# zzuiekongning/MGDT-YOLO

Measured on AMD Instinct MI355X. Metric: images/sec @640x640 bs=32 per GPU, detection forward + NMS (whole job: 1 GPU(s)), higher is better.
Workload: dtype bf16; 1 GPU; mspa_c2f_gd_yolov8-n (MSPA-C2f + GD neck + Detect, nc=80) 640x640 inference, batch 32/GPU: forward + decode + NMS(conf 0.25, iou 0.7), hipGraph replay, 4 batches in flight (one captured graph per resident batch, replayed round-robin on 4 streams); global_batch=32, parallelism=replicas x1 (batch-sharded, no data-path collective), rccl_ranks=1, input=bfloat16 NCHW images, 8 different batches resident in HBM (600 MiB) cycled, detections_last_step=9600, weights=seeded random init (no checkpoints offline), batches_in_flight=4

## Files before the change

### include/mgdt.h

```cpp
#ifndef MGDT_H
#define MGDT_H
#include <stddef.h>
#include <stdint.h>

#ifdef __cplusplus
extern "C" {
#endif

typedef void* mgdt_stream;

typedef enum { MGDT_OK = 0, MGDT_BAD_SHAPE = -1, MGDT_BAD_DTYPE = -2, MGDT_LAUNCH_FAIL = -3, MGDT_BAD_ARG = -4,
               MGDT_WORKSPACE = -5 } mgdt_status;
typedef enum { MGDT_F32 = 0, MGDT_BF16 = 1, MGDT_U8 = 2  } mgdt_dtype;
typedef enum { MGDT_ACT_NONE = 0, MGDT_ACT_SILU = 1, MGDT_ACT_RELU = 2, MGDT_ACT_GELU = 3 } mgdt_act;

typedef struct {
  void* p;
  int32_t n, h, w, c;
  int64_t sn, sh, sw, sc;
} mgdt_view;

const char* mgdt_last_error(void);
const char* mgdt_version(void);

// ... 4 lines not shown
int mgdt_conv_pack_dgrad(const float* w_oihw, int cin, int cout, int k, int phase, int dtype, void* packed_out, float* bias_out, mgdt_stream s);
typedef struct mgdt_pack_desc {
  const float* w; const float* conv_bias; const float* bn_gamma; const float* bn_beta; const float* bn_mean; const float* bn_var;
  float bn_eps; int32_t cin, cout, k, dtype, mode;
  void* packed; float* bias_out;
} mgdt_pack_desc;
int mgdt_conv_pack_batch(const mgdt_pack_desc* descs, int n, mgdt_stream s);

int mgdt_conv2d_fwd(const mgdt_view* x, const mgdt_view* x2, const float* in_scale, const float* in_shift,
                    const void* packed_w, const float* bias, int k, int stride, int act, const mgdt_view* r1,
                    const mgdt_view* r2, const mgdt_view* y, int dtype, mgdt_stream s);
size_t mgdt_conv_packed_bytes_fp8(int cin, int cout, int k);
int mgdt_conv_pack_fp8(const float* w_oihw, const float* conv_bias, const float* bn_gamma, const float* bn_beta, const float* bn_mean,
                       const float* bn_var, float bn_eps, int cin, int cout, int k, float x_qscale, void* packed_out, float* bias_out,
                       float* oscale_out, mgdt_stream s);
int mgdt_conv2d_fp8_fwd(const mgdt_view* x, const mgdt_view* x2, const float* in_scale, const float* in_shift, const void* packed_w,
                        const float* bias, const float* oscale, float x_qscale, int k, int stride, int act, const mgdt_view* r1,
                        const mgdt_view* r2, const mgdt_view* y, mgdt_stream s);
enum { MGDT_ROUTE_X2 = 1, MGDT_ROUTE_IN_SCALE = 2, MGDT_ROUTE_IN_SHIFT = 4, MGDT_ROUTE_R1 = 8, MGDT_ROUTE_R2 = 16, MGDT_ROUTE_FP8 = 32 };
enum { MGDT_ROUTE_IGEMM = 0, MGDT_ROUTE_LDS3X3 = 1 };
typedef struct {
  int32_t family, nchunks, waves, lds_bytes;
  int32_t NT, MT, D, extra, nseg, seg_chunks, gx, gy, numTiles, ragged;
  int32_t NBW, tile_rows, ncg, nwg, ntiles;
} mgdt_conv_route;
int mgdt_conv2d_route(const mgdt_view* x, const mgdt_view* y, int k, int stride, int dtype, int flags, int act, mgdt_conv_route* out);
int mgdt_conv2d_phase_fwd(const mgdt_view* x, const void* packed_w, const float* bias, int phase, const mgdt_view* r1, const mgdt_view* r2,
                          const mgdt_view* y, int dtype, mgdt_stream s);

size_t mgdt_cnx_mlp_packed_bytes(int c, int dtype);
int mgdt_cnx_mlp_pack(const float* w1, const float* b1, const float* w2, const float* b2, int c, void* packed, int dtype, mgdt_stream s);
size_t mgdt_cnx_mlp_workspace_bytes(int n, int h, int w, int c);
int mgdt_cnx_mlp_fwd(const mgdt_view* t, const mgdt_view* res, const void* packed, const float* gamma, const float* beta, void* ws,
                     const mgdt_view* y, int dtype, mgdt_stream s);

int mgdt_cnx_block_supported(int n, int h, int w, int c, int dtype);
size_t mgdt_cnx_block_workspace_bytes(int n, int h, int w, int c);
int mgdt_cnx_block_geometry(int h, int w, int c, int* out);
int mgdt_cnx_block_fwd(const mgdt_view* x, const float* dw_w49c, const float* dw_b, const float* ln_w, const float* ln_b, float eps, const void* packed,
                       const float* gamma, const float* beta, const void* tail_w, const float* tail_b, int tail_act, void* ws, size_t ws_bytes,
                       const mgdt_view* y, int dtype, mgdt_stream s);

size_t mgdt_stem2_packed_bytes(void);
int mgdt_stem2_pack(const float* w_folded, void* packed, mgdt_stream s);
int mgdt_stem2_fwd(const mgdt_view* x, int x_dtype, const void* packed0, const float* bias0, const void* packed1, const float* bias1,
                   const mgdt_view* y, mgdt_stream s);
int mgdt_stem2_geometry(int n, int h, int w, int cu_count, int* out);
int mgdt_stem2_route(const mgdt_view* x, int x_dtype, const mgdt_view* y, int cu_count, int* out);

int mgdt_detect_tail_supported(int c2, int c3, int nc, int reg_max, int dtype);
int mgdt_detect_tail_fwd(const mgdt_view* tb, const mgdt_view* tc, const void* wb, const float* bb, const void* wc, const float* bc, int nc,
                         float stride, int a_off, int a_total, const mgdt_view* feat, float* y, unsigned long long* best_keys,
                         const void* wb3, const float* bb3, mgdt_stream s);
int mgdt_detect_tail_aug_fwd(const mgdt_view* tb, const mgdt_view* tc, const void* wb, const float* bb, const void* wc, const float* bc, int nc,
                             float stride, int a_off, int a_total, const mgdt_view* feat, float* y, unsigned long long* best_keys,
                             const void* wb3, const float* bb3, float aug_scale, int aug_flip, float aug_img_w, mgdt_stream s);

int mgdt_scale_img_fwd(const mgdt_view* x, int x_dtype, int flip, int hs, int ws, float pad, const mgdt_view* y, int y_dtype, mgdt_stream s);

int mgdt_csp_block_supported(int mode, int cin, int cout, int wd, int nbtl, int h, int w, int dtype);
int mgdt_csp_block_tiles(int mode, int n, int cin, int cout, int wd, int nbtl, int h, int w, int* geom8);
int mgdt_csp_block_fwd(int mode, const mgdt_view* x, const void* front, const float* front_bias, const void* const* mid,
                       const float* const* mid_bias, int nbtl, int shortcut, const void* back, const float* back_bias, int wd, int act,
                       const mgdt_view* y, float* pool, int dtype, mgdt_stream s);

size_t mgdt_pw_chain_packed_bytes(int wd, int dtype);
int mgdt_pw_chain_pack(int idx, const float* w_oi, const float* conv_bias, const float* bn_gamma, const float* bn_beta, const float* bn_mean,
                       const float* bn_var, float bn_eps, int wd, int dtype, void* packed, mgdt_stream s);
int mgdt_pw_chain3_fwd(const mgdt_view* x, const void* packed, int wd, int act, const mgdt_view* y, int dtype, mgdt_stream s);

int mgdt_conv1x1_inject_supported(int cin, int cout, int h, int w, int hg, int wg, int dtype);
int mgdt_conv1x1_inject_fwd(const mgdt_view* x, const void* packed_w, const float* bias, const mgdt_view* ga, const mgdt_view* gf,
                            const mgdt_view* y, int dtype, mgdt_stream s);

int mgdt_conv1x1_inject_conv_supported(int cin, int cmid, int cout2, int h, int w, int hg, int wg, int dtype);
int mgdt_conv1x1_inject_conv_fwd(const mgdt_view* x, const void* packed_w, const float* bias, const mgdt_view* ga, const mgdt_view* gf,
                                 const mgdt_view* gsrc, const void* packed_wg, const float* bias_g, int cmid,
                                 const void* packed_w2, const float* bias2, int act2, const mgdt_view* y2, int dtype, mgdt_stream s);

size_t mgdt_groupnorm_workspace_bytes(int n, int c);
int mgdt_groupnorm_fwd(const mgdt_view* x, const float* gamma, const float* beta, int groups, float eps, int act, void* ws, const mgdt_view* y,
                       int dtype, mgdt_stream s);
int mgdt_tood_layer_attn_fwd(const float* sums, int n, int c, int hw, const float* w1, const float* b1, const float* w2, const float* b2, int hid,
                             int stacked, float* scale, mgdt_stream s);
int mgdt_dcnv2_fwd(const mgdt_view* x, const mgdt_view* offset_mask, const float* w_gemm, const float* bias, const mgdt_view* y, int dtype,
                   mgdt_stream s);
int mgdt_dcnv2_mfma_fwd(const mgdt_view* x, const mgdt_view* offset_mask, const void* packed_w, const mgdt_view* y, int dtype, mgdt_stream s);
int mgdt_pixel_gate_fwd(const mgdt_view* x, const mgdt_view* gate, const mgdt_view* y, int dtype, mgdt_stream s);

int mgdt_conv_pack_direct(const float* w_oihw, const float* conv_bias, const float* bn_gamma, const float* bn_beta,
                          const float* bn_mean, const float* bn_var, float bn_eps, int cin_g, int cout, int k,
                          float* w_out, float* bias_out, mgdt_stream s);
int mgdt_conv2d_direct_fwd(const mgdt_view* x, int x_dtype, const float* w_gemm, const float* bias, int k, int stride,
                           int groups, int act, const mgdt_view* y, int dtype, mgdt_stream s);
enum { MGDT_DIRECT_STEM = 0, MGDT_DIRECT_GENERIC = 1, MGDT_DIRECT_REFUSED = 2 };
int mgdt_conv2d_direct_route(const mgdt_view* x, int x_dtype, const mgdt_view* y, int dtype, int k, int stride, int groups, int* out);

#define MGDT_SPR_SPLITS 16
int mgdt_spr_pool_fwd(const mgdt_view* x, float* pooled, int dtype, mgdt_stream s);
int mgdt_spr_attn_fwd(const float* pooled, const float* fc1_w, const float* fc1_b, const float* fc2_w,
                      const float* fc2_b, int n, int c, int groups, int h, int w, int softmax, float* attn, mgdt_stream s);
int mgdt_scale_channels_fwd(const mgdt_view* x, const float* attn, const mgdt_view* y, int dtype, mgdt_stream s);
int mgdt_spr_attn_scale_fwd(const float* pooled, int nsplit, int tiles_x, int tiles_y, const float* fc1_w, const float* fc1_b, const float* fc2_w, const float* fc2_b, int groups,
                            const mgdt_view* x, const mgdt_view* y, const mgdt_view* pool_a, const mgdt_view* pool_b, int dtype, mgdt_stream s);

int mgdt_sppf_pool_fwd(const mgdt_view* x, const mgdt_view* y1, const mgdt_view* y2, const mgdt_view* y3, int dtype,
// ... 234 lines not shown
```

### mgdt_yolo_amd/_lib.py

```python
import ctypes as C
import os

_HERE = os.path.dirname(os.path.abspath(__file__))
LIB_PATH = os.environ.get('MGDT_LIB') or os.path.join(_HERE, 'csrc', 'libmgdt_hip.so')

F32, BF16 = 0, 1
ACT_NONE, ACT_SILU, ACT_RELU, ACT_GELU = 0, 1, 2, 3
SPR_SPLITS = 16
GRN_SPLITS = 8


class View(C.Structure):
    _fields_ = [('p', C.c_void_p), ('n', C.c_int32), ('h', C.c_int32), ('w', C.c_int32), ('c', C.c_int32),
                ('sn', C.c_int64), ('sh', C.c_int64), ('sw', C.c_int64), ('sc', C.c_int64)]


VP = C.POINTER(View)
_vp, _i, _f, _sz, _l = C.c_void_p, C.c_int, C.c_float, C.c_size_t, C.c_long

class PackDesc(C.Structure):
    _fields_ = [('w', C.c_void_p), ('conv_bias', C.c_void_p), ('bn_gamma', C.c_void_p), ('bn_beta', C.c_void_p), ('bn_mean', C.c_void_p), ('bn_var', C.c_void_p),
                ('bn_eps', C.c_float), ('cin', C.c_int32), ('cout', C.c_int32), ('k', C.c_int32), ('dtype', C.c_int32), ('mode', C.c_int32),
                ('packed', C.c_void_p), ('bias_out', C.c_void_p)]


class WgradFinalDesc(C.Structure):
    _fields_ = [('partial', C.c_void_p), ('dw', C.c_void_p), ('n', C.c_long), ('nsplit', C.c_int32), ('accumulate', C.c_int32)]


class ConvRoute(C.Structure):
    _fields_ = [(n, C.c_int32) for n in ('family', 'nchunks', 'waves', 'lds_bytes', 'NT', 'MT', 'D', 'extra', 'nseg', 'seg_chunks', 'gx', 'gy', 'numTiles',
                                         'ragged', 'NBW', 'tile_rows', 'ncg', 'nwg', 'ntiles')]


ROUTE_X2, ROUTE_IN_SCALE, ROUTE_IN_SHIFT, ROUTE_R1, ROUTE_R2, ROUTE_FP8 = 1, 2, 4, 8, 16, 32
ROUTE_IGEMM, ROUTE_LDS3X3 = 0, 1
DIRECT_STEM, DIRECT_GENERIC, DIRECT_REFUSED = 0, 1, 2

PROTOTYPES = {
    'mgdt_last_error': (C.c_char_p, []),
    'mgdt_version': (C.c_char_p, []),
    'mgdt_conv_packed_bytes': (_sz, [_i, _i, _i, _i]),
    'mgdt_conv_pack': (_i, [_vp, _vp, _vp, _vp, _vp, _vp, _f, _i, _i, _i, _i, _vp, _vp, _vp]),
    'mgdt_conv2d_fwd': (_i, [VP, VP, _vp, _vp, _vp, _vp, _i, _i, _i, VP, VP, VP, _i, _vp]),
    'mgdt_conv_packed_bytes_fp8': (_sz, [_i, _i, _i]),
    'mgdt_conv_pack_fp8': (_i, [_vp, _vp, _vp, _vp, _vp, _vp, _f, _i, _i, _i, _f, _vp, _vp, _vp, _vp]),
    'mgdt_conv2d_fp8_fwd': (_i, [VP, VP, _vp, _vp, _vp, _vp, _vp, _f, _i, _i, _i, VP, VP, VP, _vp]),
    'mgdt_conv2d_route': (_i, [VP, VP, _i, _i, _i, _i, _i, C.POINTER(ConvRoute)]),
    'mgdt_conv_pack_batch': (_i, [_vp, _i, _vp]),
    'mgdt_conv2d_phase_fwd': (_i, [VP, _vp, _vp, _i, VP, VP, VP, _i, _vp]),
    'mgdt_conv_wgrad_splits': (_i, [_i, _i, _i]),
    'mgdt_wgrad_final_batch': (_i, [_vp, _i, _vp]),
    'mgdt_conv_pack_dgrad': (_i, [_vp, _i, _i, _i, _i, _i, _vp, _vp, _vp]),
    'mgdt_conv_pack_direct': (_i, [_vp, _vp, _vp, _vp, _vp, _vp, _f, _i, _i, _i, _vp, _vp, _vp]),
    'mgdt_conv2d_direct_fwd': (_i, [VP, _i, _vp, _vp, _i, _i, _i, _i, VP, _i, _vp]),
    'mgdt_conv2d_direct_route': (_i, [VP, _i, VP, _i, _i, _i, _i, C.POINTER(C.c_int)]),
    'mgdt_spr_pool_fwd': (_i, [VP, _vp, _i, _vp]),
    'mgdt_spr_attn_fwd': (_i, [_vp, _vp, _vp, _vp, _vp, _i, _i, _i, _i, _i, _i, _vp, _vp]),
    'mgdt_scale_channels_fwd': (_i, [VP, _vp, VP, _i, _vp]),
    'mgdt_sppf_pool_fwd': (_i, [VP, VP, VP, VP, _i, _vp]),
    'mgdt_adaptive_avgpool_fwd': (_i, [VP, VP, _i, _vp]),
    'mgdt_bilinear_fwd': (_i, [VP, VP, _i, _vp]),
    'mgdt_nearest_fwd': (_i, [VP, VP, _i, _vp]),
    'mgdt_copy_fwd': (_i, [VP, _i, VP, _i, _vp]),
    'mgdt_image_pad4_fwd': (_i, [VP, _i, VP, _i, _vp]),
    'mgdt_dwconv7_ln_fwd': (_i, [VP, _vp, _vp, _vp, _vp, _f, VP, _i, _vp]),
    'mgdt_cnx_mlp_packed_bytes': (_sz, [_i, _i]),
    'mgdt_cnx_mlp_pack': (_i, [_vp, _vp, _vp, _vp, _i, _vp, _i, _vp]),
    'mgdt_cnx_mlp_workspace_bytes': (_sz, [_i, _i, _i, _i]),
    'mgdt_cnx_mlp_fwd': (_i, [VP, VP, _vp, _vp, _vp, _vp, VP, _i, _vp]),
    'mgdt_cnx_block_supported': (_i, [_i, _i, _i, _i, _i]),
    'mgdt_cnx_block_workspace_bytes': (_sz, [_i, _i, _i, _i]),
    'mgdt_cnx_block_geometry': (_i, [_i, _i, _i, C.POINTER(C.c_int)]),
    'mgdt_cnx_block_fwd': (_i, [VP, _vp, _vp, _vp, _vp, _f, _vp, _vp, _vp, _vp, _vp, _i, _vp, _sz, VP, _i, _vp]),
    'mgdt_pw_chain_packed_bytes': (_sz, [_i, _i]),
    'mgdt_pw_chain_pack': (_i, [_i, _vp, _vp, _vp, _vp, _vp, _vp, _f, _i, _i, _vp, _vp]),
    'mgdt_pw_chain3_fwd': (_i, [VP, _vp, _i, _i, VP, _i, _vp]),
    'mgdt_conv1x1_inject_supported': (_i, [_i, _i, _i, _i, _i, _i, _i]),
    'mgdt_conv1x1_inject_fwd': (_i, [VP, _vp, _vp, VP, VP, VP, _i, _vp]),
    'mgdt_conv1x1_inject_conv_supported': (_i, [_i, _i, _i, _i, _i, _i, _i, _i]),
    'mgdt_conv1x1_inject_conv_fwd': (_i, [VP, _vp, _vp, VP, VP, VP, _vp, _vp, _i, _vp, _vp, _i, VP, _i, _vp]),
    'mgdt_spr_attn_scale_fwd': (_i, [_vp, _i, _i, _i, _vp, _vp, _vp, _vp, _i, VP, VP, VP, VP, _i, _vp]),
    'mgdt_stem2_packed_bytes': (_sz, []),
    'mgdt_stem2_pack': (_i, [_vp, _vp, _vp]),
    'mgdt_stem2_fwd': (_i, [VP, _i, _vp, _vp, _vp, _vp, VP, _vp]),
    'mgdt_stem2_geometry': (_i, [_i, _i, _i, _i, C.POINTER(C.c_int)]),
    'mgdt_stem2_route': (_i, [VP, _i, VP, _i, C.POINTER(C.c_int)]),
    'mgdt_detect_tail_supported': (_i, [_i, _i, _i, _i, _i]),
    'mgdt_detect_tail_fwd': (_i, [VP, VP, _vp, _vp, _vp, _vp, _i, _f, _i, _i, VP, _vp, _vp, _vp, _vp, _vp]),
    'mgdt_detect_tail_aug_fwd': (_i, [VP, VP, _vp, _vp, _vp, _vp, _i, _f, _i, _i, VP, _vp, _vp, _vp, _vp, _f, _i, _f, _vp]),
    'mgdt_scale_img_fwd': (_i, [VP, _i, _i, _i, _i, _f, VP, _i, _vp]),
    'mgdt_csp_block_supported': (_i, [_i, _i, _i, _i, _i, _i, _i, _i]),
    'mgdt_csp_block_tiles': (_i, [_i, _i, _i, _i, _i, _i, _i, _i, _vp]),
    'mgdt_csp_block_fwd': (_i, [_i, VP, _vp, _vp, _vp, _vp, _i, _i, _vp, _vp, _i, _i, VP, _vp, _i, _vp]),
    'mgdt_groupnorm_workspace_bytes': (_sz, [_i, _i]),
    'mgdt_groupnorm_fwd': (_i, [VP, _vp, _vp, _i, _f, _i, _vp, VP, _i, _vp]),
    'mgdt_tood_layer_attn_fwd': (_i, [_vp, _i, _i, _i, _vp, _vp, _vp, _vp, _i, _i, _vp, _vp]),
    'mgdt_dcnv2_fwd': (_i, [VP, VP, _vp, _vp, VP, _i, _vp]),
    'mgdt_dcnv2_mfma_fwd': (_i, [VP, VP, _vp, VP, _i, _vp]),
    'mgdt_pixel_gate_fwd': (_i, [VP, VP, VP, _i, _vp]),
    'mgdt_gn_affine': (_i, [_vp, _vp, _i, _i, _i, _vp, _vp, _i, _f, _vp, _vp, _vp, _vp, _vp]),
    'mgdt_nc_affine_act_bwd': (_i, [VP, VP, _vp, _vp, _i, VP, _i, _vp]),
    'mgdt_gn_bwd_workspace_bytes': (_sz, [_i, _i]),
    'mgdt_gn_bwd_coef': (_i, [_vp, _vp, _vp, _vp, _vp, _i, _i, _i, _i, _vp, _vp, _vp, _vp, _vp, _i, _vp, _vp]),
    'mgdt_nc_axpby': (_i, [VP, _vp, VP, _vp, _vp, VP, _i, _vp]),
    'mgdt_pixel_gate_bwd': (_i, [VP, VP, VP, VP, VP, _i, _vp]),
    'mgdt_tood_layer_attn_bwd_workspace_bytes': (_sz, [_i, _i, _i, _i]),
    'mgdt_tood_layer_attn_bwd': (_i, [_vp, _vp, _i, _i, _i, _vp, _vp, _vp, _vp, _i, _i, _vp, _vp, _vp, _vp, _vp, _i, _vp, _vp]),
    'mgdt_dcn_im2col': (_i, [VP, VP, VP, _i, _vp]),
    'mgdt_dcn_col2im_bwd': (_i, [VP, VP, VP, _vp, VP, _i, _vp]),
    'mgdt_val_match_fwd': (_i, [_vp, _vp, _i, _i, _vp, _vp, _i, _vp, _i, _vp, _vp]),
    'mgdt_grn_stats_fwd': (_i, [VP, _vp, _vp, _vp, _i, _vp]),
    'mgdt_dwconv7_ln_route': (_i, [_i, _i, _i, _i, _i, C.POINTER(C.c_int)]),
    'mgdt_inject_fwd': (_i, [VP, VP, VP, VP, _i, _vp]),
    'mgdt_detect_decode_fwd': (_i, [VP, _i, _i, _f, _i, _i, _vp, _i, _vp]),
    'mgdt_detect_decode_aug_fwd': (_i, [VP, _i, _i, _f, _i, _i, _vp, _vp, _f, _i, _f, _i, _vp]),
    'mgdt_detect_loss_workspace_bytes': (_sz, [_i, _i, _i]),
    'mgdt_detect_loss_fwd': (_i, [_vp, _vp, _i, _i, _i, _vp, _i, _i, _f, _f, _f, _vp, _vp, _vp, _vp, _vp, _sz, _i, _vp]),
    'mgdt_detect_loss_fwd_dev': (_i, [_vp, _vp, _i, _i, _i, _vp, _i, _vp, _f, _f, _f, _vp, _vp, _vp, _vp, _vp, _sz, _i, _vp]),
    'mgdt_detect_loss_bwd': (_i, [_vp, _vp, _vp, _i, _i, _i, _vp, _i, _f, _f, _f, _f, _vp, _vp, _sz, _i, _vp]),
    'mgdt_reduce_workspace_bytes': (_sz, [_i]),
    'mgdt_bn_stats_fwd': (_i, [VP, _f, _f, _vp, _vp, _vp, _vp, _vp, _i, _vp]),
    'mgdt_bn_act_fwd': (_i, [VP, _vp, _vp, _vp, _vp, _i, VP, VP, VP, _i, _vp]),
    'mgdt_bn_act_bwd': (_i, [VP, VP, _vp, _vp, _vp, _vp, _i, _vp, _vp, VP, _vp, _i, _vp]),
    'mgdt_conv_dgrad': (_i, [VP, _vp, _i, _i, VP, _i, _i, _vp]),
    'mgdt_gconv_dgrad': (_i, [VP, _vp, _i, _i, _i, VP, _i, _i, _vp]),
    'mgdt_gconv_wgrad_workspace_bytes': (_sz, [_i, _i, _i, _i]),
    'mgdt_gconv_wgrad': (_i, [VP, VP, _i, _i, _i, _vp, _i, _vp, _i, _vp]),
    'mgdt_conv_wgrad_workspace_bytes': (_sz, [_i, _i, _i]),
    'mgdt_conv_wgrad': (_i, [VP, VP, VP, _i, _i, _vp, _vp, _i, _vp, _i, _vp]),
    'mgdt_add_fwd': (_i, [VP, VP, VP, _i, _vp]),
    'mgdt_maxpool5_bwd': (_i, [VP, VP, _vp, _i, _vp]),
    'mgdt_nearest_bwd': (_i, [VP, VP, _i, _vp]),
    'mgdt_ew_binary': (_i, [VP, VP, VP, _i, _i, _vp]),
    'mgdt_channel_affine': (_i, [VP, _vp, _vp, VP, _i, _vp]),
    'mgdt_nc_reduce_workspace_bytes': (_sz, [_i, _i]),
    'mgdt_nc_reduce': (_i, [VP, VP, _vp, _vp, _i, _vp]),
    'mgdt_adaptive_avgpool_bwd': (_i, [VP, VP, _i, _i, _vp]),
    'mgdt_bilinear_bwd': (_i, [VP, VP, _i, _i, _vp]),
    'mgdt_spr_bwd_workspace_bytes': (_sz, [_i, _i, _i]),
    'mgdt_spr_bwd': (_i, [VP, _vp, _i, _vp, _vp, _vp, _vp, _vp, _vp, _i, VP, _vp, _vp, _i, _vp]),
    'mgdt_dwconv7_ln_train_fwd': (_i, [VP, _vp, _vp, _vp, _vp, _f, VP, VP, _i, _vp]),
    'mgdt_dwconv7_ln_bwd_workspace_bytes': (_sz, [_i]),
# ... 86 lines not shown
```

### mgdt_yolo_amd/csrc/detect_tail.hip

```cpp
#include "conv_igemm_kernel.h"

struct DtArgs {
  const char* tb; int bsn, bsh, bsw; uint32_t tb_bytes;
  const char* tc; int csn, csh, csw; uint32_t tc_bytes;
  char* feat; int fsn, fsh, fsw; uint32_t feat_bytes;
  const char* wb; const float* bb; const char* wc; const float* bc;
  float* y;
  unsigned long long* best;
  const char* wb3; const float* bb3;
  int N, H, W, HW, c2, c3, nc, kch, nbc, units_per_img, units, a_off, a_total;
  float stride;
  FastDiv fd_w;
  int aug, aug_flip;
  float aug_s, aug_w;
};

constexpr int DT_THREADS = 256;
constexpr int DT_P = 20;
constexpr int DT_WT = (2 * 16 + 4) * DT_P;

__global__ __launch_bounds__(DT_THREADS) void detect_tail_kernel(const DtArgs a) {
  extern __shared__ __attribute__((aligned(16))) char smem[];
  char* wbl = smem;
  char* wcl = smem + 1024;
  float* biasl = (float*)(wcl + (size_t)a.kch * a.nbc * 1024);
  float* ytile = biasl + 16 + a.nbc * 16;
  char* wb3l = (char*)(ytile + (size_t)4 * DT_WT);
  float* bias3l = (float*)(wb3l + 5 * 1024);
  const int tid = threadIdx.x, lane = tid & 63;
  const int wave = __builtin_amdgcn_readfirstlane(tid >> 6);
  const int r = lane & 15, g = lane >> 4;
  for (int i = tid; i < 64; i += DT_THREADS) ((uint4*)wbl)[i] = ((const uint4*)a.wb)[i];
  for (int i = tid; i < a.kch * a.nbc * 64; i += DT_THREADS) ((uint4*)wcl)[i] = ((const uint4*)a.wc)[i];
  for (int i = tid; i < 16 + a.nbc * 16; i += DT_THREADS) biasl[i] = i < 16 ? a.bb[i] : a.bc[i - 16];
  if (a.wb3) {
    for (int i = tid; i < 5 * 64; i += DT_THREADS) ((uint4*)wb3l)[i] = ((const uint4*)a.wb3)[i];
    if (tid < 16) bias3l[tid] = a.bb3[tid];
  }
  __syncthreads();
  const __amdgpu_buffer_rsrc_t brs = __builtin_amdgcn_make_buffer_rsrc((void*)a.tb, 0, a.tb_bytes, 0x00020000);
  const __amdgpu_buffer_rsrc_t crs = __builtin_amdgcn_make_buffer_rsrc((void*)a.tc, 0, a.tc_bytes, 0x00020000);
  const __amdgpu_buffer_rsrc_t frs = __builtin_amdgcn_make_buffer_rsrc((void*)a.feat, 0, a.feat_bytes, 0x00020000);
  float* yt = ytile + (size_t)wave * DT_WT;
  const char* wlane_b = wbl + lane * 16;
  const char* wlane_c = wcl + lane * 16;
  const int boff = (8 * g < a.c2) ? g * 16 : MGDT_OOB;
  const int r4 = 16;

  const bool vec_ok = (a.HW & 3) == 0 && (a.a_off & 3) == 0 && (a.a_total & 3) == 0 && ((uintptr_t)a.y & 15) == 0;
  auto wave_sync = [&]() __attribute__((always_inline)) {
    __builtin_amdgcn_fence(__ATOMIC_RELEASE, "wavefront");
    __builtin_amdgcn_wave_barrier();
    __builtin_amdgcn_fence(__ATOMIC_ACQUIRE, "wavefront");
  };
  auto flush = [&](const float* tile, int nrow, int row0, int n, int an0) __attribute__((always_inline)) {
    const int row = lane >> 2, q = (lane & 3) * 4;
    if (row < nrow && row0 + row < 4 + a.nc) {
      float* dst = a.y + ((size_t)n * (4 + a.nc) + row0 + row) * a.a_total + a.a_off + an0 + q;
      const float* src = tile + row * DT_P + q;
      if (vec_ok) { if (an0 + q < a.HW) *(f32x4*)dst = *(const f32x4*)src; }
      else {
#pragma unroll
        for (int e = 0; e < 4; ++e) if (an0 + q + e < a.HW) dst[e] = src[e];
      }
    }
  };
  int flip = 0;
  for (int unit = blockIdx.x * 4 + wave; unit < a.units; unit += gridDim.x * 4) {
    const int n = unit / a.units_per_img, a0 = (unit - n * a.units_per_img) * 32;
    float bs[2] = {-1.f, -1.f};
    int bcl[2] = {0, 0};
#pragma unroll
    for (int u = 0; u < 2; ++u) {
      const int an = a0 + u * 16 + r;
      const bool pv = an < a.HW;
      const int oy = (int)fdiv((uint32_t)(pv ? an : 0), a.fd_w), ox = (pv ? an : 0) - oy * a.W;
      const int bo = pv ? n * a.bsn + oy * a.bsh + ox * a.bsw : MGDT_OOB;
      const int co = pv ? n * a.csn + oy * a.csh + ox * a.csw : MGDT_OOB;
      const int fo = pv ? n * a.fsn + oy * a.fsh + ox * a.fsw : MGDT_OOB;
      bf16x8 Bb;
      if (a.wb3) {
        bf16x8 B3[5];
#pragma unroll
        for (int kc = 0; kc < 5; ++kc) {
          const int p = kc * 4 + g, tap = p >> 1, cp = p & 1;
          const int iy = oy + tap / 3 - 1, ix = ox + tap % 3 - 1;
          const bool ok = pv && tap < 9 && (unsigned)iy < (unsigned)a.H && (unsigned)ix < (unsigned)a.W;
          B3[kc] = __builtin_bit_cast(bf16x8, __builtin_amdgcn_raw_buffer_load_b128(brs, ok ? (uint32_t)(n * a.bsn + iy * a.bsh + ix * a.bsw + cp * 16) : (uint32_t)MGDT_OOB, 0, 0));
        }
        f32x4 acc3 = *(const f32x4*)(bias3l + 4 * g);
#pragma unroll
// ... 30 lines not shown
      const float x1 = ax - dl, y1 = ay - dt, x2 = ax + dr, y2 = ay + db;
      float comp = g == 0 ? (x1 + x2) / 2.f * a.stride : g == 1 ? (y1 + y2) / 2.f * a.stride : g == 2 ? (x2 - x1) * a.stride : (y2 - y1) * a.stride;
      if (a.aug) {
        comp = comp / a.aug_s;
        if (g == 0 && a.aug_flip) comp = a.aug_w - comp;
      }
      {
        float* bt = yt + 32 * DT_P;
        bt[g * DT_P + r] = comp;
        wave_sync();
        flush(bt, 4, 0, n, a0 + u * 16);
      }
      for (int nb = 0; nb < a.nbc; ++nb) {
        f32x4 acc = *(const f32x4*)(biasl + 16 + nb * 16 + 4 * g);
#pragma unroll
        for (int kc = 0; kc < 4; ++kc)
          if (kc < a.kch) acc = mma(*(const bf16x8*)(wlane_c + (size_t)(kc * a.nbc + nb) * 1024), Bc[kc], acc);
        const int c = nb * 16 + 4 * g;
        float lc[4];
#pragma unroll
        for (int j = 0; j < 4; ++j) lc[j] = (float)(bf16)acc[j];
        bstore4<bf16>(frs, c < a.nc ? (uint32_t)fo + (uint32_t)((r4 + c) * 2) : (uint32_t)MGDT_OOB, f32x4{lc[0], lc[1], lc[2], lc[3]});
        float* ct = yt + flip * 16 * DT_P;
        flip ^= 1;
#pragma unroll
        for (int j = 0; j < 4; ++j) {
          const float sg = fast_sigmoid(lc[j]);
          ct[(4 * g + j) * DT_P + r] = sg;
          if (c + j < a.nc && sg > bs[u]) { bs[u] = sg; bcl[u] = c + j; }
        }
        wave_sync();
        flush(ct, 16, 4 + nb * 16, n, a0 + u * 16);
      }
    }
    if (a.best) {
#pragma unroll
      for (int u = 0; u < 2; ++u) {
#pragma unroll
        for (int off = 16; off <= 32; off <<= 1) {
          const float os = __shfl_xor(bs[u], off, 64);
          const int oc = __shfl_xor(bcl[u], off, 64);
          if (os > bs[u] || (os == bs[u] && oc < bcl[u])) { bs[u] = os; bcl[u] = oc; }
        }
        if (g == 0 && a0 + u * 16 + r < a.HW) {
          const unsigned an = (unsigned)(a.a_off + a0 + u * 16 + r);
          a.best[(size_t)n * a.a_total + an] = ((unsigned long long)(0xFFFFFFFFu - __float_as_uint(bs[u])) << 32) | (unsigned long long)(an * (unsigned)a.nc + (unsigned)bcl[u]);
        }
      }
    }
    wave_sync();
  }
}

extern "C" int mgdt_detect_tail_supported(int c2, int c3, int nc, int reg_max, int dtype) {
  return dtype == MGDT_BF16 && reg_max == 4 && c2 % 8 == 0 && c2 <= 32 && c3 % 8 == 0 && c3 <= 128 && nc >= 4 && nc <= 256 && nc % 4 == 0;
}

static int detect_tail_launch(const mgdt_view* tb, const mgdt_view* tc, const void* wb, const float* bb, const void* wc, const float* bc, int nc,
                              float stride, int a_off, int a_total, const mgdt_view* feat, float* y, unsigned long long* best_keys,
                              const void* wb3, const float* bb3, bool aug, float aug_scale, int aug_flip, float aug_img_w, mgdt_stream s) {
  if (!view_ok(tb) || !view_ok(tc) || !view_ok(feat) || !wb || !bb || !wc || !bc || !y) MGDT_FAIL(MGDT_BAD_ARG, "detect_tail: null/empty argument");
  if (!mgdt_detect_tail_supported(tb->c, tc->c, nc, 4, MGDT_BF16)) MGDT_FAIL(MGDT_BAD_SHAPE, "detect_tail: c2=%d c3=%d nc=%d not covered", tb->c, tc->c, nc);
  if (feat->c != 16 + nc || tb->n != tc->n || tb->h != tc->h || tb->w != tc->w || feat->n != tb->n || feat->h != tb->h || feat->w != tb->w ||
      a_off < 0 || a_off + tb->h * tb->w > a_total)
    MGDT_FAIL(MGDT_BAD_SHAPE, "detect_tail: shapes");
  DtArgs a;
  memset(&a, 0, sizeof(a));
  bool fits = true;
  auto bind = [&](const mgdt_view* v, const char** p, int* sn, int* sh, int* sw, uint32_t* bytes, int q) {
    const long ext = ((long)(v->n - 1) * v->sn + (long)(v->h - 1) * v->sh + (long)(v->w - 1) * v->sw + v->c) * 2;
    if (v->sc != 1 || v->sw % q || v->sh % q || v->sn % q || (uintptr_t)v->p % (q * 2) || ext >= 0x7fffffffL) { fits = false; return; }
    *p = (const char*)v->p; *sn = (int)(v->sn * 2); *sh = (int)(v->sh * 2); *sw = (int)(v->sw * 2); *bytes = (uint32_t)ext;
  };
  const char* fp = nullptr;
  bind(tb, &a.tb, &a.bsn, &a.bsh, &a.bsw, &a.tb_bytes, 8);
  bind(tc, &a.tc, &a.csn, &a.csh, &a.csw, &a.tc_bytes, 8);
  bind(feat, &fp, &a.fsn, &a.fsh, &a.fsw, &a.feat_bytes, 4);
  if (!fits) MGDT_FAIL(MGDT_BAD_SHAPE, "detect_tail: views must be 16-byte aligned NHWC (sc == 1) below 2 GiB");
  a.feat = (char*)fp;
  a.wb = (const char*)wb; a.bb = bb; a.wc = (const char*)wc; a.bc = bc; a.y = y; a.best = best_keys;
  a.wb3 = (const char*)wb3; a.bb3 = bb3;
  if (wb3 && (!bb3 || tb->c != 16)) MGDT_FAIL(MGDT_BAD_SHAPE, "detect_tail: the in-launch 3x3 box conv is built for 16 -> 16 channels");
  a.N = tb->n; a.H = tb->h; a.W = tb->w; a.HW = tb->h * tb->w; a.c2 = tb->c; a.c3 = tc->c; a.nc = nc;
  a.kch = cdiv(tc->c, 32); a.nbc = cdiv(nc, 16);
  a.units_per_img = cdiv(a.HW, 32); a.units = a.N * a.units_per_img;
  a.a_off = a_off; a.a_total = a_total; a.stride = stride; a.fd_w = make_fastdiv((uint32_t)tb->w);
  a.aug = aug ? 1 : 0; a.aug_flip = aug_flip ? 1 : 0; a.aug_s = aug_scale; a.aug_w = aug_img_w;
  const size_t lds = 1024 + (size_t)a.kch * a.nbc * 1024 + (size_t)(16 + a.nbc * 16) * 4 + (size_t)4 * DT_WT * 4 + 5 * 1024 + 64;
  if (lds > 150 * 1024) MGDT_FAIL(MGDT_BAD_SHAPE, "detect_tail: nc=%d needs %zu B of LDS", nc, lds);
  static size_t attr = 0;
  if (lds > 64 * 1024 && lds > attr) {
    hipError_t e = hipFuncSetAttribute((const void*)detect_tail_kernel, hipFuncAttributeMaxDynamicSharedMemorySize, 150 * 1024);
    if (e != hipSuccess) MGDT_FAIL(MGDT_LAUNCH_FAIL, "detect_tail: hipFuncSetAttribute: %s", hipGetErrorString(e));
    attr = 150 * 1024;
  }
  const int grid = std::min(cdiv(a.units, 4), 1024);
  detect_tail_kernel<<<grid, DT_THREADS, lds, (hipStream_t)s>>>(a);
  MGDT_CHECK_LAUNCH("detect_tail_fwd");
  return MGDT_OK;
}

extern "C" int mgdt_detect_tail_fwd(const mgdt_view* tb, const mgdt_view* tc, const void* wb, const float* bb, const void* wc, const float* bc, int nc,
                                    float stride, int a_off, int a_total, const mgdt_view* feat, float* y, unsigned long long* best_keys,
                                    const void* wb3, const float* bb3, mgdt_stream s) {
  return detect_tail_launch(tb, tc, wb, bb, wc, bc, nc, stride, a_off, a_total, feat, y, best_keys, wb3, bb3, false, 1.f, 0, 0.f, s);
}

extern "C" int mgdt_detect_tail_aug_fwd(const mgdt_view* tb, const mgdt_view* tc, const void* wb, const float* bb, const void* wc, const float* bc, int nc,
                                        float stride, int a_off, int a_total, const mgdt_view* feat, float* y, unsigned long long* best_keys,
                                        const void* wb3, const float* bb3, float aug_scale, int aug_flip, float aug_img_w, mgdt_stream s) {
  if (!(aug_scale > 0.f)) MGDT_FAIL(MGDT_BAD_ARG, "detect_tail_aug: scale %g", (double)aug_scale);
  return detect_tail_launch(tb, tc, wb, bb, wc, bc, nc, stride, a_off, a_total, feat, y, best_keys, wb3, bb3, true, aug_scale, aug_flip, aug_img_w, s);
}
```

### mgdt_yolo_amd/ops.py

```python
import ctypes as C
import os

import numpy as np
import torch

from . import _lib as L
from ._lib import ACT_GELU, ACT_NONE, ACT_RELU, ACT_SILU, BF16, F32, View

U8 = 2
_DT = {torch.float32: F32, torch.bfloat16: BF16}


def dtype_code(dt):
    try:
        return _DT[dt]
    except KeyError:
        raise RuntimeError(f'mgdt_yolo_amd computes in float32 or bfloat16, not {dt}') from None


def _need_gpu(t):
    if not t.is_cuda:
        raise RuntimeError('mgdt_yolo_amd runs on MI355X (HIP) only: got a CPU tensor and there is no CPU/PyTorch fallback')


# ... 702 lines not shown
def dcn_col2im_bwd(gcol, x, om, gom=None):
    b, c, h, w = x.shape
    gx32 = torch.zeros(b, h, w, c, dtype=torch.float32, device=x.device)
    gom = like(om) if gom is None else gom
    _same(gcol, x, om, gom)
    _launch('dcn_col2im_bwd', 'mgdt_dcn_col2im_bwd', vp(gcol), vp(x), vp(om), ptr(gx32), vp(gom), dtype_code(x.dtype), stream())
    gx = gx32.permute(0, 3, 1, 2)
    return (gx if x.dtype == torch.float32 else copy(gx, like(x))), gom


def ew_add_nc(a, b):
    return a + b


def inject(local, ga, gf, out=None):
    out = like(local) if out is None else out
    _same(local, ga, gf, out)
    _launch('inject_fwd', 'mgdt_inject_fwd', vp(local), vp(ga), vp(gf), vp(out), dtype_code(local.dtype), stream())
    return out


def detect_decode(feat, reg_max, nc, stride, a_off, y, aug=None, best=None):
    if aug is None:
        _launch('detect_decode_fwd', 'mgdt_detect_decode_fwd', vp(feat), reg_max, nc, float(stride), a_off, y.shape[2], ptr(y), dtype_code(feat.dtype),
                stream())
        return
    s, flip, img_w = aug
    _launch('detect_decode_aug_fwd', 'mgdt_detect_decode_aug_fwd', vp(feat), reg_max, nc, float(stride), a_off, y.shape[2], ptr(y), ptr(best), float(s),
            int(bool(flip)), float(img_w), dtype_code(feat.dtype), stream())


FUSED_DETECT_TAIL = True


def detect_tail_supported(tb, tc, nc, reg_max, dtype):
    return bool(FUSED_DETECT_TAIL and dtype == torch.bfloat16 and tb.dtype == dtype and tc.dtype == dtype and is_nhwc(tb) and is_nhwc(tc) and
                L.lib().mgdt_detect_tail_supported(tb.shape[1], tc.shape[1], int(nc), int(reg_max), dtype_code(dtype)))


FUSED_DETECT_BOX3 = True


def detect_tail(tb, tc, pkb, pkc, nc, stride, a_off, feat, y, best=None, pk3=None, aug=None):
    if _PROF is not None:
        b, _, h, w = tb.shape
        _META['detect_tail_fwd'] = dict(shape=(b, tb.shape[1] + tc.shape[1], h, w, 16 + nc, 1, 1), flops=2.0 * b * h * w * (tb.shape[1] * 16 + tc.shape[1] * nc),
                                        bytes=float((tb.numel() + tc.numel() + feat.numel()) * 2 + b * (4 + nc) * h * w * 4))
    args = (vp(tb), vp(tc), ptr(pkb.w), ptr(pkb.bias), ptr(pkc.w), ptr(pkc.bias), int(nc), float(stride), int(a_off), y.shape[2], vp(feat), ptr(y), ptr(best),
            None if pk3 is None else ptr(pk3.w), None if pk3 is None else ptr(pk3.bias))
    if aug is None:
        _launch('detect_tail_fwd', 'mgdt_detect_tail_fwd', *args, stream())
    else:
        _launch('detect_tail_aug_fwd', 'mgdt_detect_tail_aug_fwd', *args, float(aug[0]), int(bool(aug[1])), float(aug[2]), stream())


TTA_PAD = 0.447


def scale_img(x, hs, ws, hp, wp, flip, dtype):
    _need_gpu(x)
    y = torch.empty(x.shape[0], 3, hp, wp, dtype=dtype, device=x.device)
    if _PROF is not None:
        _META['scale_img_fwd'] = dict(shape=(x.shape[0], 3, x.shape[2], x.shape[3], 3, hp, wp), flops=0.0,
                                      bytes=float(x.numel() * x.element_size() + y.numel() * y.element_size()))
    _launch('scale_img_fwd', 'mgdt_scale_img_fwd', vp(x), U8 if x.dtype == torch.uint8 else dtype_code(x.dtype), int(bool(flip)), int(hs), int(ws),
            float(TTA_PAD), vp(y), dtype_code(dtype), stream())
    return y


NMS_USE_BEST_KEYS = True


def attach_best_keys(y, best):
    y._mgdt_best = (best, y._version)


def _best_keys_of(pred, b, a):
    bk = getattr(pred, '_mgdt_best', None)
    if not NMS_USE_BEST_KEYS or bk is None:
        return None
    best, ver = bk
    if ver != pred._version or best.shape != (b, a) or best.dtype != torch.int64 or best.device != pred.device or not best.is_contiguous():
        return None
    return best
def nms(pred, conf_thres, iou_thres, classes, agnostic, multi_label, max_det, max_nms, max_wh):
    _need_gpu(pred)
    if pred.dtype != torch.float32 or not pred.is_contiguous():
        raise RuntimeError('nms: prediction must be a contiguous float32 tensor')
    b, ch, a = pred.shape
    nc = ch - 4
    lib = L.lib()
    ml = 1 if (multi_label and nc > 1) else 0
    ws_bytes = lib.mgdt_nms_workspace_bytes(b, nc, a, ml, max_nms)
    ws = torch.empty(max(ws_bytes, 8), dtype=torch.uint8, device=pred.device)
    out = torch.empty(b, max_det, 6, dtype=torch.float32, device=pred.device)
    kept = torch.empty(b, max_det, dtype=torch.int32, device=pred.device)
    counts = torch.empty(b, dtype=torch.int32, device=pred.device)
    cls_t = None
    if classes is not None:
        cls_t = torch.as_tensor(list(classes), dtype=torch.int32).to(pred.device)
    best = None if ml else _best_keys_of(pred, b, a)
    _launch('nms_fwd', 'mgdt_nms_fwd', ptr(pred), b, nc, a, float(conf_thres), float(iou_thres), ptr(cls_t), 0 if cls_t is None else cls_t.numel(),
                             int(bool(agnostic)), ml, max_det, max_nms, float(max_wh), ptr(out), ptr(kept), ptr(counts), ptr(best), ptr(ws),
                             ws_bytes, stream())
    return out, kept, counts

# ... 1264 lines not shown
```

Before: 41150 images/sec.

## Add fixed-shape detect tail kernel with software-pipelined loads and buffer stores

Adds a specialized detect-tail kernel for the common head shape (c2=16, c3 in 3 chunks, nc=80, fused 3x3 box conv, best-keys) that issues the next unit's global loads before the current unit's epilogue. It also writes outputs through buffer stores and uses an occupancy launch bound. Weight panel staging into LDS is batched into unrolled 8-wide loads to expose more memory parallelism, and grid sizing is routed through a plan helper. This aims to hide global load latency in the detect tail at the cost of more registers and a narrower code path, with a generic fallback.

Result: no change. 41410 images/sec (median of 6 runs) (+0.6%).

```diff
diff --git a/include/mgdt.h b/include/mgdt.h
--- a/include/mgdt.h
+++ b/include/mgdt.h
@@ -80,6 +80,8 @@
 int mgdt_detect_tail_fwd(const mgdt_view* tb, const mgdt_view* tc, const void* wb, const float* bb, const void* wc, const float* bc, int nc,
                          float stride, int a_off, int a_total, const mgdt_view* feat, float* y, unsigned long long* best_keys,
                          const void* wb3, const float* bb3, mgdt_stream s);
+enum { MGDT_TAIL_GENERIC = 0, MGDT_TAIL_FIXED = 1 };
+int mgdt_detect_tail_route(const mgdt_view* tb, const mgdt_view* tc, int nc, int a_off, int a_total, const void* y, int box3, int best, int aug, int* out);
 int mgdt_detect_tail_aug_fwd(const mgdt_view* tb, const mgdt_view* tc, const void* wb, const float* bb, const void* wc, const float* bc, int nc,
                              float stride, int a_off, int a_total, const mgdt_view* feat, float* y, unsigned long long* best_keys,
                              const void* wb3, const float* bb3, float aug_scale, int aug_flip, float aug_img_w, mgdt_stream s);
diff --git a/mgdt_yolo_amd/_lib.py b/mgdt_yolo_amd/_lib.py
--- a/mgdt_yolo_amd/_lib.py
+++ b/mgdt_yolo_amd/_lib.py
@@ -36,6 +36,7 @@
 ROUTE_X2, ROUTE_IN_SCALE, ROUTE_IN_SHIFT, ROUTE_R1, ROUTE_R2, ROUTE_FP8 = 1, 2, 4, 8, 16, 32
 ROUTE_IGEMM, ROUTE_LDS3X3 = 0, 1
 DIRECT_STEM, DIRECT_GENERIC, DIRECT_REFUSED = 0, 1, 2
+TAIL_GENERIC, TAIL_FIXED = 0, 1
 
 PROTOTYPES = {
     'mgdt_last_error': (C.c_char_p, []),
@@ -89,6 +90,7 @@
     'mgdt_detect_tail_supported': (_i, [_i, _i, _i, _i, _i]),
     'mgdt_detect_tail_fwd': (_i, [VP, VP, _vp, _vp, _vp, _vp, _i, _f, _i, _i, VP, _vp, _vp, _vp, _vp, _vp]),
     'mgdt_detect_tail_aug_fwd': (_i, [VP, VP, _vp, _vp, _vp, _vp, _i, _f, _i, _i, VP, _vp, _vp, _vp, _vp, _f, _i, _f, _vp]),
+    'mgdt_detect_tail_route': (_i, [VP, VP, _i, _i, _i, _vp, _i, _i, _i, C.POINTER(C.c_int)]),
     'mgdt_scale_img_fwd': (_i, [VP, _i, _i, _i, _i, _f, VP, _i, _vp]),
     'mgdt_csp_block_supported': (_i, [_i, _i, _i, _i, _i, _i, _i, _i]),
     'mgdt_csp_block_tiles': (_i, [_i, _i, _i, _i, _i, _i, _i, _i, _vp]),
diff --git a/mgdt_yolo_amd/csrc/detect_tail.hip b/mgdt_yolo_amd/csrc/detect_tail.hip
--- a/mgdt_yolo_amd/csrc/detect_tail.hip
+++ b/mgdt_yolo_amd/csrc/detect_tail.hip
@@ -10,7 +10,8 @@
   const char* wb3; const float* bb3;
   int N, H, W, HW, c2, c3, nc, kch, nbc, units_per_img, units, a_off, a_total;
   float stride;
-  FastDiv fd_w;
+  FastDiv fd_w, fd_upi;
+  uint32_t y_bytes;
   int aug, aug_flip;
   float aug_s, aug_w;
 };
@@ -18,6 +19,27 @@
 constexpr int DT_THREADS = 256;
 constexpr int DT_P = 20;
 constexpr int DT_WT = (2 * 16 + 4) * DT_P;
+#ifndef DT_AHEAD
+#define DT_AHEAD 1
+#endif
+
+__device__ __forceinline__ void dt_stage_panels(const DtArgs& a, char* wbl, char* wcl, char* wb3l, int ncls, int n3, int tid) {
+  const int total = 64 + ncls + n3;
+  for (int i0 = tid; i0 < total; i0 += 8 * DT_THREADS) {
+    uint4 t[8];
+#pragma unroll
+    for (int u = 0; u < 8; ++u) {
+      const int i = min(i0 + u * DT_THREADS, total - 1);
+      const uint4* src = i < 64 ? (const uint4*)a.wb + i : i < 64 + ncls ? (const uint4*)a.wc + (i - 64) : (const uint4*)a.wb3 + (i - 64 - ncls);
+      t[u] = *src;
+    }
+#pragma unroll
+    for (int u = 0; u < 8; ++u) {
+      const int i = i0 + u * DT_THREADS;
+      if (i < total) *(i < 64 ? (uint4*)wbl + i : i < 64 + ncls ? (uint4*)wcl + (i - 64) : (uint4*)wb3l + (i - 64 - ncls)) = t[u];
+    }
+  }
+}
 
 __global__ __launch_bounds__(DT_THREADS) void detect_tail_kernel(const DtArgs a) {
   extern __shared__ __attribute__((aligned(16))) char smem[];
@@ -30,13 +52,9 @@
   const int tid = threadIdx.x, lane = tid & 63;
   const int wave = __builtin_amdgcn_readfirstlane(tid >> 6);
   const int r = lane & 15, g = lane >> 4;
-  for (int i = tid; i < 64; i += DT_THREADS) ((uint4*)wbl)[i] = ((const uint4*)a.wb)[i];
-  for (int i = tid; i < a.kch * a.nbc * 64; i += DT_THREADS) ((uint4*)wcl)[i] = ((const uint4*)a.wc)[i];
+  dt_stage_panels(a, wbl, wcl, wb3l, a.kch * a.nbc * 64, a.wb3 ? 5 * 64 : 0, tid);
   for (int i = tid; i < 16 + a.nbc * 16; i += DT_THREADS) biasl[i] = i < 16 ? a.bb[i] : a.bc[i - 16];
-  if (a.wb3) {
-    for (int i = tid; i < 5 * 64; i += DT_THREADS) ((uint4*)wb3l)[i] = ((const uint4*)a.wb3)[i];
-    if (tid < 16) bias3l[tid] = a.bb3[tid];
-  }
+  if (a.wb3 && tid < 16) bias3l[tid] = a.bb3[tid];
   __syncthreads();
   const __amdgpu_buffer_rsrc_t brs = __builtin_amdgcn_make_buffer_rsrc((void*)a.tb, 0, a.tb_bytes, 0x00020000);
   const __amdgpu_buffer_rsrc_t crs = __builtin_amdgcn_make_buffer_rsrc((void*)a.tc, 0, a.tc_bytes, 0x00020000);
@@ -173,8 +191,225 @@
   }
 }
 
+#ifndef DT_NT
+#define DT_NT 1
+#endif
+__device__ __forceinline__ bf16x4 dt_round4(f32x4 v, float* w) {
+  bf16x4 o;
+#pragma unroll
+  for (int i = 0; i < 4; ++i) o[i] = (bf16)v[i];
+  const auto pk = __builtin_bit_cast(__attribute__((__vector_size__(2 * sizeof(unsigned int)))) unsigned int, o);
+  w[0] = __uint_as_float(pk[0] << 16); w[1] = __uint_as_float(pk[0] & 0xffff0000u);
+  w[2] = __uint_as_float(pk[1] << 16); w[3] = __uint_as_float(pk[1] & 0xffff0000u);
+  return o;
+}
+__device__ __forceinline__ void dt_store_map(__amdgpu_buffer_rsrc_t rs, uint32_t off, bf16x4 o) {
+  __builtin_amdgcn_raw_buffer_store_b64(__builtin_bit_cast(__attribute__((__vector_size__(2 * sizeof(unsigned int)))) unsigned int, o), rs, off, 0, (DT_NT & 2) ? 2 : 0);
+}
+
+template <int KCH> struct DtLoads { bf16x8 t[5]; bf16x8 c[KCH]; int oy, ox, fo; };
+
+template <int KCH, int NBC, bool BOX3, bool BEST, int AHEAD>
+__global__ __launch_bounds__(DT_THREADS, 4) void detect_tail_fixed_kernel(const DtArgs a) {
+  static_assert(BOX3, "the fixed-shape route is built for the head with the 3x3 box conv in the launch");
+  static_assert(AHEAD == 1 || AHEAD == 2, "one group or one unit ahead");
+  constexpr int OFF_WC = 1024, OFF_BIAS = OFF_WC + KCH * NBC * 1024, OFF_YT = OFF_BIAS + (16 + NBC * 16) * 4, OFF_W3 = OFF_YT + 4 * DT_WT * 4,
+                OFF_B3 = OFF_W3 + 5 * 1024;
+  extern __shared__ __attribute__((aligned(16))) char smem[];
+  const int tid = threadIdx.x, lane = tid & 63;
+  const int wave = __builtin_amdgcn_readfirstlane(tid >> 6);
+  const int r = lane & 15, g = lane >> 4;
+  const __amdgpu_buffer_rsrc_t brs = __builtin_amdgcn_make_buffer_rsrc((void*)a.tb, 0, a.tb_bytes, 0x00020000);
+  const __amdgpu_buffer_rsrc_t crs = __builtin_amdgcn_make_buffer_rsrc((void*)a.tc, 0, a.tc_bytes, 0x00020000);
+  const __amdgpu_buffer_rsrc_t frs = __builtin_amdgcn_make_buffer_rsrc((void*)a.feat, 0, a.feat_bytes, 0x00020000);
+  const __amdgpu_buffer_rsrc_t yrs = __builtin_amdgcn_make_buffer_rsrc((void*)a.y, 0, a.y_bytes, 0x00020000);
+  int toff[5];
+  uint32_t need = 0;
+#pragma unroll
+  for (int kc = 0; kc < 5; ++kc) {
+    const int p = kc * 4 + g, tap = p >> 1, cp = p & 1, dy = tap / 3 - 1, dx = tap % 3 - 1;
+    toff[kc] = dy * a.bsh + dx * a.bsw + cp * 16;
+    need |= ((dy < 0 ? 1u : 0u) | (dy > 0 ? 2u : 0u) | (dx < 0 ? 4u : 0u) | (dx > 0 ? 8u : 0u) | 16u | (tap < 9 ? 0u : 32u)) << (6 * kc);
+  }
+  const uint32_t clast = ((KCH - 1) * 4 + g) * 8 < a.c3 ? (uint32_t)(((KCH - 1) * 4 + g) * 16) : (uint32_t)MGDT_OOB;
+
+  auto request = [&](int unit, int u) __attribute__((always_inline)) {
+    DtLoads<KCH> L;
+    const bool ex = unit < a.units;
+    const int un = ex ? unit : 0;
+    const int n = (int)fdiv((uint32_t)un, a.fd_upi), a0 = (un - n * a.units_per_img) * 32;
+    const int an = a0 + u * 16 + r;
+    const bool pv = ex && an < a.HW;
+    const int ap = pv ? an : 0;
+    L.oy = (int)fdiv((uint32_t)ap, a.fd_w);
+    L.ox = ap - L.oy * a.W;
+    const int bo = n * a.bsn + L.oy * a.bsh + L.ox * a.bsw;
+    const uint32_t bad = (L.oy == 0 ? 1u : 0u) | (L.oy == a.H - 1 ? 2u : 0u) | (L.ox == 0 ? 4u : 0u) | (L.ox == a.W - 1 ? 8u : 0u) | (pv ? 0u : 16u) | 32u;
+#pragma unroll
+    for (int kc = 0; kc < 5; ++kc) {
+      const bool ok = ((need >> (6 * kc)) & bad) == 0;
+      L.t[kc] = __builtin_bit_cast(bf16x8, __builtin_amdgcn_raw_buffer_load_b128(brs, ok ? (uint32_t)(bo + toff[kc]) : (uint32_t)MGDT_OOB, 0, 0));
+    }
+    const int co = n * a.csn + L.oy * a.csh + L.ox * a.csw;
+#pragma unroll
+    for (int kc = 0; kc < KCH; ++kc) {
+      const uint32_t off = kc < KCH - 1 ? (uint32_t)(co + (kc * 4 + g) * 16) : (uint32_t)co + clast;
+      L.c[kc] = __builtin_bit_cast(bf16x8, __builtin_amdgcn_raw_buffer_load_b128(crs, pv ? off : (uint32_t)MGDT_OOB, 0, 0));
+    }
+    L.fo = pv ? n * a.fsn + L.oy * a.fsh + L.ox * a.fsw : MGDT_OOB;
+    return L;
+  };
+
+  const int step = gridDim.x * 4;
+  int unit = blockIdx.x * 4 + wave;
+  DtLoads<KCH> S[AHEAD];
+#pragma unroll
+  for (int d = 0; d < AHEAD; ++d) S[d] = request(unit + (d >> 1) * step, d & 1);
+
+  constexpr int NBIAS = 16 + NBC * 16;
+  static_assert(NBIAS + 16 <= DT_THREADS, "one bias value per thread");
+  const float bv = tid < 16 ? a.bb[tid] : tid < NBIAS ? a.bc[tid - 16] : tid < NBIAS + 16 ? a.bb3[tid - NBIAS] : 0.f;
+  dt_stage_panels(a, smem, smem + OFF_WC, smem + OFF_W3, KCH * NBC * 64, 5 * 64, tid);
+  if (tid < NBIAS) ((float*)(smem + OFF_BIAS))[tid] = bv;
+  else if (tid < NBIAS + 16) ((float*)(smem + OFF_B3))[tid - NBIAS] = bv;
+  __syncthreads();
+
+  const char* wl = smem + lane * 16;
+  const float* biasg = (const float*)(smem + OFF_BIAS) + 4 * g;
+  const float* bias3g = (const float*)(smem + OFF_B3) + 4 * g;
+  float* yt = (float*)(smem + OFF_YT) + wave * DT_WT;
+  float* ytw = yt + 4 * g * DT_P + r;
+  const int frow = lane >> 2, fq = (lane & 3) * 4;
+  const float* ytr = yt + frow * DT_P + fq;
+  const float* ytb = yt + (32 + (frow & 3)) * DT_P + fq;
+  const int ylane = (frow * a.a_total + fq) * 4;
+  const uint32_t rows16 = (uint32_t)a.a_total * 64u;
+  auto wave_sync = [&]() __attribute__((always_inline)) {
+    __builtin_amdgcn_fence(__ATOMIC_RELEASE, "wavefront");
+    __builtin_amdgcn_wave_barrier();
+    __builtin_amdgcn_fence(__ATOMIC_ACQUIRE, "wavefront");
+  };
+  auto ystore = [&](const float* src, uint32_t voff, uint32_t soff) __attribute__((always_inline)) {
+    typedef __attribute__((__vector_size__(4 * sizeof(unsigned int)))) unsigned int u32x4;
+    __builtin_amdgcn_raw_buffer_store_b128(__builtin_bit_cast(u32x4, *(const f32x4*)src), yrs, voff, soff, (DT_NT & 1) ? 2 : 0);
+  };
+
+  for (; unit < a.units; unit += step) {
+    const int n = (int)fdiv((uint32_t)unit, a.fd_upi), a0 = (unit - n * a.units_per_img) * 32;
+    const uint32_t ybase = (uint32_t)((n * (4 + NBC * 16)) * a.a_total + a.a_off + a0) * 4u;
+#pragma unroll
+    for (int u = 0; u < 2; ++u) {
+      float bs = -1.f;
+      int bcl = 0;
+      DtLoads<KCH>& L = S[u % AHEAD];
+      const int ox = L.ox, oy = L.oy, fo = L.fo;
+      f32x4 acc3 = *(const f32x4*)bias3g;
+#pragma unroll
+      for (int kc = 0; kc < 5; ++kc) acc3 = mma(*(const bf16x8*)(wl + OFF_W3 + kc * 1024), L.t[kc], acc3);
+      bf16x8 Bb;
+#pragma unroll
+      for (int e = 0; e < 8; ++e) Bb[e] = e < 4 ? (bf16)(acc3[e] * fast_sigmoid(acc3[e])) : (bf16)0.f;
+      f32x4 accb = *(const f32x4*)biasg;
+      accb = mma(*(const bf16x8*)wl, Bb, accb);
+      float lb[4];
+      dt_store_map(frs, (uint32_t)fo + (uint32_t)(4 * g * 2), dt_round4(accb, lb));
+      const float mx = fmaxf(fmaxf(lb[0], lb[1]), fmaxf(lb[2], lb[3]));
+      float den = 0.f, num = 0.f;
+#pragma unroll
+      for (int k = 0; k < 4; ++k) {
+        const float e = __builtin_amdgcn_exp2f((lb[k] - mx) * 1.4426950408889634f);
+        den += e;
+        num += e * (float)k;
+      }
+      const float dd = num * __builtin_amdgcn_rcpf(den);
+      const float dl = __shfl(dd, r, 64), dt = __shfl(dd, 16 + r, 64), dr = __shfl(dd, 32 + r, 64), db = __shfl(dd, 48 + r, 64);
+      const float ax = (float)ox + 0.5f, ay = (float)oy + 0.5f;
+      const float x1 = ax - dl, y1 = ay - dt, x2 = ax + dr, y2 = ay + db;
+      const float comp = g == 0 ? (x1 + x2) / 2.f * a.stride : g == 1 ? (y1 + y2) / 2.f * a.stride : g == 2 ? (x2 - x1) * a.stride : (y2 - y1) * a.stride;
+      const bool qv = a0 + u * 16 + fq < a.HW;
+      const uint32_t yl = qv ? (uint32_t)ylane : (uint32_t)MGDT_OOB;
+      ytw[(32 - 3 * g) * DT_P] = comp;
+      wave_sync();
+      ystore(ytb, frow < 4 ? yl : (uint32_t)MGDT_OOB, ybase + u * 64);
+      f32x4 acc[NBC];
+#pragma unroll
+      for (int nb = 0; nb < NBC; ++nb) {
+        acc[nb] = *(const f32x4*)(biasg + 16 + nb * 16);
+#pragma unroll
+        for (int kc = 0; kc < KCH; ++kc) acc[nb] = mma(*(const bf16x8*)(wl + OFF_WC + (kc * NBC + nb) * 1024), L.c[kc], acc[nb]);
+      }
+      L = request(unit + ((u + AHEAD) >> 1) * step, (u + AHEAD) & 1);
+#pragma unroll
+      for (int nb = 0; nb < NBC; ++nb) {
+        const int c = nb * 16 + 4 * g;
+        float lc[4];
+        dt_store_map(frs, (uint32_t)fo + (uint32_t)((16 + nb * 16) * 2) + (uint32_t)(4 * g * 2), dt_round4(acc[nb], lc));
+        const int tile = ((u * NBC + nb) & 1) * 16 * DT_P;
+#pragma unroll
+        for (int j = 0; j < 4; ++j) {
+          const float sg = fast_sigmoid(lc[j]);
+          ytw[tile + j * DT_P] = sg;
+          if (BEST && sg > bs) { bs = sg; bcl = c + j; }
+        }
+        wave_sync();
+        ystore(ytr + tile, yl, ybase + u * 64 + 4 * (uint32_t)a.a_total * 4u + nb * rows16);
+      }
+      if (BEST) {
+#pragma unroll
+        for (int off = 16; off <= 32; off <<= 1) {
+          const float os = __shfl_xor(bs, off, 64);
+          const int oc = __shfl_xor(bcl, off, 64);
+          if (os > bs || (os == bs && oc < bcl)) { bs = os; bcl = oc; }
+        }
+        if (g == 0 && a0 + u * 16 + r < a.HW) {
+          const unsigned an = (unsigned)(a.a_off + a0 + u * 16 + r);
+          a.best[(size_t)n * a.a_total + an] = ((unsigned long long)(0xFFFFFFFFu - __float_as_uint(bs)) << 32) | (unsigned long long)(an * (unsigned)(NBC * 16) + (unsigned)bcl);
+        }
+      }
+    }
+    wave_sync();
+  }
+}
+
 extern "C" int mgdt_detect_tail_supported(int c2, int c3, int nc, int reg_max, int dtype) {
   return dtype == MGDT_BF16 && reg_max == 4 && c2 % 8 == 0 && c2 <= 32 && c3 % 8 == 0 && c3 <= 128 && nc >= 4 && nc <= 256 && nc % 4 == 0;
+}
+
+constexpr int DT_SLOTS = 1024;
+struct DtPlan { int route, grid, lds, units; };
+static size_t detect_tail_lds(int kch, int nbc) {
+  return 1024 + (size_t)kch * nbc * 1024 + (size_t)(16 + nbc * 16) * 4 + (size_t)4 * DT_WT * 4 + 5 * 1024 + 64;
+}
+static DtPlan detect_tail_plan(int n, int h, int w, int c2, int c3, int nc, int a_off, int a_total, const void* y, bool box3, bool best, bool aug) {
+  DtPlan p;
+  const int hw = h * w, kch = cdiv(c3, 32), nbc = cdiv(nc, 16);
+  p.units = n * cdiv(hw, 32);
+  p.lds = (int)detect_tail_lds(kch, nbc);
+  const char* er = getenv("MGDT_DETECT_TAIL_ROUTE");
+  const bool vec_ok = (hw & 3) == 0 && (a_off & 3) == 0 && (a_total & 3) == 0 && ((uintptr_t)y & 15) == 0;
+  const bool fixed = !(er && !strcmp(er, "generic")) && !aug && box3 && best && c2 == 16 && kch == 3 && nc == 80 && vec_ok &&
+                     (long)n * (4 + nc) * a_total * 4 < 0x7fffffffL;
+  p.route = fixed ? MGDT_TAIL_FIXED : MGDT_TAIL_GENERIC;
+  if (fixed) {
+    const int upw = cdiv(p.units, 4 * DT_SLOTS);
+    p.grid = cdiv(p.units, 4 * upw);
+  } else {
+    p.grid = std::min(cdiv(p.units, 4), DT_SLOTS);
+  }
+  const char* eg = getenv("MGDT_DETECT_TAIL_GRID");
+  if (eg && atoi(eg) > 0) p.grid = std::min(p.grid, atoi(eg));
+  return p;
+}
+
+extern "C" int mgdt_detect_tail_route(const mgdt_view* tb, const mgdt_view* tc, int nc, int a_off, int a_total, const void* y, int box3, int best, int aug,
+                                      int* out) {
+  if (!tb || !tc || !out) MGDT_FAIL(MGDT_BAD_ARG, "detect_tail_route: null argument");
+  if (!mgdt_detect_tail_supported(tb->c, tc->c, nc, 4, MGDT_BF16) || tb->n != tc->n || tb->h != tc->h || tb->w != tc->w || tb->n <= 0 || tb->h <= 0 ||
+      tb->w <= 0 || a_off < 0 || a_off + tb->h * tb->w > a_total)
+    MGDT_FAIL(MGDT_BAD_SHAPE, "detect_tail_route: shapes");
+  const DtPlan p = detect_tail_plan(tb->n, tb->h, tb->w, tb->c, tc->c, nc, a_off, a_total, y, box3 != 0, best != 0, aug != 0);
+  out[0] = p.route; out[1] = p.grid; out[2] = p.lds; out[3] = p.units;
+  return MGDT_OK;
 }
 
 static int detect_tail_launch(const mgdt_view* tb, const mgdt_view* tc, const void* wb, const float* bb, const void* wc, const float* bc, int nc,
@@ -207,7 +442,15 @@
   a.units_per_img = cdiv(a.HW, 32); a.units = a.N * a.units_per_img;
   a.a_off = a_off; a.a_total = a_total; a.stride = stride; a.fd_w = make_fastdiv((uint32_t)tb->w);
   a.aug = aug ? 1 : 0; a.aug_flip = aug_flip ? 1 : 0; a.aug_s = aug_scale; a.aug_w = aug_img_w;
-  const size_t lds = 1024 + (size_t)a.kch * a.nbc * 1024 + (size_t)(16 + a.nbc * 16) * 4 + (size_t)4 * DT_WT * 4 + 5 * 1024 + 64;
+  a.fd_upi = make_fastdiv((uint32_t)a.units_per_img);
+  const DtPlan plan = detect_tail_plan(a.N, a.H, a.W, a.c2, a.c3, nc, a_off, a_total, y, wb3 != nullptr, best_keys != nullptr, aug);
+  const size_t lds = (size_t)plan.lds;
+  if (plan.route == MGDT_TAIL_FIXED) {
+    a.y_bytes = (uint32_t)((long)a.N * (4 + nc) * a_total * 4);
+    detect_tail_fixed_kernel<3, 5, true, true, DT_AHEAD><<<plan.grid, DT_THREADS, lds, (hipStream_t)s>>>(a);
+    MGDT_CHECK_LAUNCH("detect_tail_fwd");
+    return MGDT_OK;
+  }
   if (lds > 150 * 1024) MGDT_FAIL(MGDT_BAD_SHAPE, "detect_tail: nc=%d needs %zu B of LDS", nc, lds);
   static size_t attr = 0;
   if (lds > 64 * 1024 && lds > attr) {
@@ -215,8 +458,7 @@
     if (e != hipSuccess) MGDT_FAIL(MGDT_LAUNCH_FAIL, "detect_tail: hipFuncSetAttribute: %s", hipGetErrorString(e));
     attr = 150 * 1024;
   }
-  const int grid = std::min(cdiv(a.units, 4), 1024);
-  detect_tail_kernel<<<grid, DT_THREADS, lds, (hipStream_t)s>>>(a);
+  detect_tail_kernel<<<plan.grid, DT_THREADS, lds, (hipStream_t)s>>>(a);
   MGDT_CHECK_LAUNCH("detect_tail_fwd");
   return MGDT_OK;
 }
diff --git a/mgdt_yolo_amd/ops.py b/mgdt_yolo_amd/ops.py
--- a/mgdt_yolo_amd/ops.py
+++ b/mgdt_yolo_amd/ops.py
@@ -778,6 +778,13 @@
         _launch('detect_tail_fwd', 'mgdt_detect_tail_fwd', *args, stream())
     else:
         _launch('detect_tail_aug_fwd', 'mgdt_detect_tail_aug_fwd', *args, float(aug[0]), int(bool(aug[1])), float(aug[2]), stream())
+
+
+def detect_tail_route(tb, tc, nc, a_off, y, best=None, pk3=None, aug=None):
+    out = (C.c_int * 4)()
+    L.check(L.lib().mgdt_detect_tail_route(vp(tb), vp(tc), int(nc), int(a_off), y.shape[2], ptr(y), int(pk3 is not None), int(best is not None),
+                                           int(aug is not None), out), 'detect_tail_route')
+    return dict(route='fixed' if out[0] == L.TAIL_FIXED else 'generic', grid=out[1], lds_bytes=out[2], units=out[3])
 
 
 TTA_PAD = 0.447
```
